# bentotten/radiation_ppo

Hardware: AMD Instinct MI355X
Metric: env steps/sec (whole node) at 4096 envs; PPO iters/sec at 1/2/4/8 GPUs (higher is better)
Workload: dtype f32 policy / f64+int32 env

## Files before the change

### include/radsearch.h

```cpp
#ifndef RADSEARCH_H
#define RADSEARCH_H

#include <stddef.h>
#include <stdint.h>

#ifdef __cplusplus
extern "C" {
#endif

#define RS_ABI_VERSION 4
#define RS_OBS_DIM 11
#define RS_NUM_ACTIONS 9
#define RS_MAX_AGENTS 8
#define RS_MAX_OBS 7

typedef void* rs_stream_t;
typedef struct rs_handle rs_handle;

enum {
    RS_OK = 0,
    RS_ERR_INVALID_ARG = 1,
    RS_ERR_HIP = 2,
    RS_ERR_WORKSPACE = 3,
    RS_ERR_UNSUPPORTED = 4
// ... 22 lines not shown
    int32_t debug_spawn;
} rs_config;

typedef struct rs_info {
    uint8_t* out_of_bounds;
    int32_t* out_of_bounds_count;
    uint8_t* blocked;
    uint8_t* collision;
} rs_info;

const char* rs_strerror(int code);
int rs_abi_version(void);

size_t rs_state_bytes(const rs_config* cfg);

int rs_create(const rs_config* cfg, void* workspace, size_t workspace_bytes, rs_stream_t stream, rs_handle** out);
void rs_destroy(rs_handle* h);

int rs_state_field(rs_handle* h, const char* name, void** dev_ptr, int32_t* elem_bytes, int32_t* rows, int32_t* cols);

int rs_set_epoch_end(rs_handle* h, rs_stream_t stream);

int rs_reset(rs_handle* h, const uint8_t* mask, float* obs, float* reward, float* team, uint8_t* done,
             const rs_info* info, rs_stream_t stream);

int rs_refresh(rs_handle* h, const uint8_t* mask, const int32_t* src_xy, const int32_t* det_xy, const int32_t* intensity,
               const int32_t* bkg, const int32_t* num_obs, const int32_t* rects, float* obs, float* reward, float* team,
               uint8_t* done, const rs_info* info, rs_stream_t stream);

int rs_step(rs_handle* h, const int8_t* actions, float* obs, float* reward, float* team, uint8_t* done,
            const rs_info* info, rs_stream_t stream);

int rs_action_uniforms(rs_handle* h, float* u, rs_stream_t stream);

int rs_error_flags(rs_handle* h, rs_stream_t stream, uint32_t* flags_out);

int rs_gae(const float* rew, const float* val, const uint8_t* cut, const float* last_val, float* adv, float* ret,
           int32_t T, int32_t M, double gamma, double lam, rs_stream_t stream);

size_t rs_ppo_prepare_workspace_bytes(int32_t N);
int rs_ppo_prepare(const uint8_t* cut, const float* adv, float* w, float* adv_n, float* mean_std, void* workspace, int32_t T, int32_t N,
                   int32_t n_total, rs_stream_t stream);

typedef struct rs_mlp_params {
    const float *w1, *b1, *w2, *b2, *w3, *b3;
} rs_mlp_params;

int rs_policy_forward(const rs_mlp_params* actor, const rs_mlp_params* critic, const float* x, int32_t M,
                      float* logits, float* value, rs_stream_t stream);

int rs_ff_team_step(const rs_mlp_params* actors, const rs_mlp_params* critics, int32_t num_agents, const float* x, const float* u,
                    int64_t* act, float* logp_val_boot, int8_t* act8, const uint8_t* mask, int32_t num_envs, rs_stream_t stream);

typedef struct rs_rollout_args {
    int32_t steps_per_epoch;
    int32_t steps_per_episode;
    float* obs;
    int64_t* act;
    float* logp;
    float* val;
    float* rew;
    float* last_val;
    uint8_t* cut;
    float* source_tar;
    float* cur_obs;
    double* w_count;
// ... 306 lines not shown
```

### radiation_ppo_amd/_lib.py

```python
import ctypes as C
import os

import torch

_PKG = os.path.dirname(os.path.abspath(__file__))
LIB_PATH = os.environ.get("RS_LIB_PATH") or os.path.join(_PKG, "lib", "librs_hip.so")

RS_OBS_DIM = 11
RS_MAX_AGENTS = 8
RS_MAX_OBS = 7

ENVERR_ZERO_DIST = 1
ENVERR_IDLE_STALL = 2
ENVERR_CORRECT_CAP = 4
ENVERR_BAD_ACTION = 8
ENVERR_NO_PATH = 16

MAPERR_RING_FULL = 1
MAPERR_VISIT_OVERFLOW = 2
MAPERR_OFF_MAP = 4


class RsConfig(C.Structure):
    _fields_ = [
# ... 44 lines not shown
class RsRolloutArgs(C.Structure):
    _fields_ = [("steps_per_epoch", C.c_int32), ("steps_per_episode", C.c_int32)] + [
        (n, C.c_void_p) for n in ("obs", "act", "logp", "val", "rew", "last_val", "cut", "source_tar", "cur_obs", "w_count",
                                  "w_mean", "w_sq", "w_std", "steps_in_ep", "ep_ret", "done_count", "oob_count",
                                  "ep_ret_sum", "ep_len_sum", "ep_count", "ep_ret_sq_sum", "ep_ret_max", "ep_ret_min")]


class RsPpoBatch(C.Structure):
    _fields_ = [("x", C.c_void_p), ("act", C.c_void_p), ("adv", C.c_void_p), ("ret", C.c_void_p), ("logp_old", C.c_void_p),
                ("w", C.c_void_p), ("M", C.c_int32), ("clip_ratio", C.c_float), ("alpha", C.c_float), ("vf_coef", C.c_float)]


class RsInfo(C.Structure):
    _fields_ = [("out_of_bounds", C.c_void_p), ("out_of_bounds_count", C.c_void_p), ("blocked", C.c_void_p),
                ("collision", C.c_void_p)]


SYMBOLS = [
    ("rs_strerror", C.c_char_p, [C.c_int]),
    ("rs_abi_version", C.c_int, []),
    ("rs_state_bytes", C.c_size_t, [C.POINTER(RsConfig)]),
    ("rs_create", C.c_int, [C.POINTER(RsConfig), C.c_void_p, C.c_size_t, C.c_void_p, C.POINTER(C.c_void_p)]),
    ("rs_destroy", None, [C.c_void_p]),
    ("rs_state_field", C.c_int, [C.c_void_p, C.c_char_p, C.POINTER(C.c_void_p), C.POINTER(C.c_int32),
                                 C.POINTER(C.c_int32), C.POINTER(C.c_int32)]),
    ("rs_set_epoch_end", C.c_int, [C.c_void_p, C.c_void_p]),
    ("rs_reset", C.c_int, [C.c_void_p, C.c_void_p, C.c_void_p, C.c_void_p, C.c_void_p, C.c_void_p,
                           C.POINTER(RsInfo), C.c_void_p]),
    ("rs_refresh", C.c_int, [C.c_void_p, C.c_void_p, C.c_void_p, C.c_void_p, C.c_void_p, C.c_void_p, C.c_void_p, C.c_void_p,
                             C.c_void_p, C.c_void_p, C.c_void_p, C.c_void_p, C.POINTER(RsInfo), C.c_void_p]),
    ("rs_step", C.c_int, [C.c_void_p, C.c_void_p, C.c_void_p, C.c_void_p, C.c_void_p, C.c_void_p,
                          C.POINTER(RsInfo), C.c_void_p]),
    ("rs_action_uniforms", C.c_int, [C.c_void_p, C.c_void_p, C.c_void_p]),
    ("rs_error_flags", C.c_int, [C.c_void_p, C.c_void_p, C.POINTER(C.c_uint32)]),
    ("rs_policy_forward", C.c_int, [C.POINTER(RsMlpParams), C.POINTER(RsMlpParams), C.c_void_p, C.c_int32, C.c_void_p,
                                    C.c_void_p, C.c_void_p]),
    ("rs_ff_team_step", C.c_int, [C.POINTER(RsMlpParams), C.POINTER(RsMlpParams), C.c_int32, C.c_void_p, C.c_void_p, C.c_void_p,
                                  C.c_void_p, C.c_void_p, C.c_void_p, C.c_int32, C.c_void_p]),
    ("rs_rollout", C.c_int, [C.c_void_p, C.POINTER(RsMlpParams), C.POINTER(RsMlpParams), C.POINTER(RsRolloutArgs), C.c_void_p]),
    ("rs_ppo_grad_workspace_bytes", C.c_size_t, []),
    ("rs_ppo_grad", C.c_int, [C.POINTER(RsMlpParams), C.POINTER(RsMlpParams), C.POINTER(RsPpoBatch), C.c_void_p, C.c_void_p,
                              C.c_void_p, C.c_void_p, C.c_void_p]),
    ("rs_adam_step", C.c_int, [C.POINTER(RsMlpParams), C.POINTER(RsMlpParams), C.c_void_p, C.c_void_p, C.c_void_p, C.c_void_p,
                               C.c_void_p, C.c_float, C.c_float, C.c_void_p]),
    ("rs_ppo_update_step", C.c_int, [C.POINTER(RsMlpParams), C.POINTER(RsMlpParams), C.POINTER(RsPpoBatch), C.c_void_p, C.c_void_p,
                                     C.c_void_p, C.c_void_p, C.c_void_p, C.c_void_p, C.c_float, C.c_float, C.c_void_p]),
    ("rs_maps_state_bytes", C.c_size_t, [C.c_int32, C.c_int32, C.c_int32, C.c_int32, C.c_int32]),
    ("rs_maps_create", C.c_int, [C.c_int32, C.c_int32, C.c_int32, C.c_int32, C.c_int32, C.c_double, C.c_void_p, C.c_void_p,
                                 C.c_size_t, C.c_void_p, C.POINTER(C.c_void_p)]),
    ("rs_maps_destroy", None, [C.c_void_p]),
    ("rs_maps_reset", C.c_int, [C.c_void_p, C.c_void_p, C.c_void_p]),
    ("rs_maps_update", C.c_int, [C.c_void_p, C.c_void_p, C.c_void_p, C.c_void_p, C.c_void_p, C.c_void_p]),
    ("rs_maps_stack", C.c_int, [C.c_void_p, C.c_void_p, C.c_void_p, C.c_void_p]),
    ("rs_maps_field", C.c_int, [C.c_void_p, C.c_char_p, C.POINTER(C.c_void_p), C.POINTER(C.c_int32), C.POINTER(C.c_int32),
                                C.POINTER(C.c_int32)]),
    ("rs_cnn_trunk_slab_row", C.c_int32, [C.c_int32]),
    ("rs_cnn_trunk_slab_rows", C.c_int32, [C.c_int64, C.c_int32]),
    ("rs_cnn_trunk_scratch_floats", C.c_int32, [C.c_int32]),
    ("rs_cnn_trunk_forward", C.c_int, [C.c_void_p, C.c_void_p, C.c_void_p, C.c_int32, C.c_int32, C.c_int64, C.c_void_p, C.c_void_p,
                                       C.c_void_p, C.c_void_p, C.c_void_p, C.c_void_p, C.c_void_p, C.c_void_p, C.c_void_p, C.c_void_p]),
    ("rs_cnn_trunk_backward", C.c_int, [C.c_void_p, C.c_void_p, C.c_void_p, C.c_int32, C.c_int32, C.c_int64, C.c_void_p, C.c_void_p,
                                        C.c_void_p, C.c_void_p, C.c_void_p, C.c_void_p, C.c_void_p, C.c_void_p]),
    ("rs_gae", C.c_int, [C.c_void_p, C.c_void_p, C.c_void_p, C.c_void_p, C.c_void_p, C.c_void_p, C.c_int32,
                         C.c_int32, C.c_double, C.c_double, C.c_void_p]),
    ("rs_ppo_prepare_workspace_bytes", C.c_size_t, [C.c_int32]),
    ("rs_ppo_prepare", C.c_int, [C.c_void_p] * 6 + [C.c_int32, C.c_int32, C.c_int32, C.c_void_p]),
# ... 119 lines not shown
```

### radiation_ppo_amd/csrc/rs_device.hpp

```cpp
#pragma once
#include <hip/hip_runtime.h>
#include <stdint.h>

#include "rs_tables.hpp"

#define RS_WAVE 64
#define RS_OBS_DIM 11
#define RS_MAX_AGENTS 8
#define RS_MAX_OBS 7
#define RS_MAX_VERT (4 * RS_MAX_OBS)
#define RS_IDLE 8
#define RS_ACT_NONE 9
#define RS_CORRECT_CAP 4096

#define RS_ENVERR_ZERO_DIST 1u
#define RS_ENVERR_IDLE_STALL 2u
#define RS_ENVERR_CORRECT_CAP 4u
#define RS_ENVERR_BAD_ACTION 8u
#define RS_ENVERR_NO_PATH 16u

#define RS_AF_BLOCKED 1
#define RS_AF_INTERSECT 2
#define RS_AF_OOB 4
#define RS_AF_COLLISION 8
// ... 83 lines not shown
    const double lhs = log(v * invalpha / (a / (us * us) + b));
    const double x = k + 1.0;
    double rhs;
    if (x >= 10.0) {
        const double xi = 1.0 / x, xi2 = xi * xi;
        const double ser = xi * (0.083333333333333333 - xi2 * (0.0027777777777777778 - xi2 * (0.00079365079365079365 - xi2 * 0.00059523809523809524)));
        rhs = k * log(lam / x) - 0.5 * log(x) - lam + x - 0.91893853320467274 - ser;
    } else {
        rhs = -lam + k * log(lam) - lgamma(x);
    }
    return lhs <= rhs;
}

__device__ __forceinline__ int64_t rs_poisson(double lam, uint32_t t, uint32_t episode, uint32_t stream, uint32_t k0, uint32_t k1) {
    if (lam == 0.0) return 0;
    if (lam < 10.0) return rs_poisson_small(lam, t, episode, stream, k0, k1);
    double slam = sqrt(lam);
    double b = 0.931 + 2.53 * slam;
    double a = -0.059 + 0.02483 * b;
    double vr = 0.9277 - 3.6224 / (b - 2.0);
    for (uint32_t i = 0;; ++i) {
        u32x4 o = philox4x32_10(i, t, episode, stream, k0, k1);
        double u = u53(o.x, o.y) - 0.5;
        double v = u53(o.z, o.w);
        double us = 0.5 - fabs(u);
        if (!(us > 0.0)) continue;
        double k = floor((2.0 * a / us + b) * u + lam + 0.43);
        if (us >= 0.07 && v <= vr) return (int64_t)k;
        if (k < 0.0 || (us < 0.013 && v > us)) continue;
        if (rs_ptrs_slow_accept(v, us, k, lam, a, b)) return (int64_t)k;
    }
}

__device__ __forceinline__ double rs_round2(double x) {
    uint64_t bits = (uint64_t)__double_as_longlong(x);
    int ex = (int)((bits >> 52) & 0x7ff);
    if (ex == 0x7ff) return x;
    double sgn = (bits >> 63) ? -1.0 : 1.0;
    if (ex == 0) return sgn * 0.0;
    uint64_t m = (bits & 0xFFFFFFFFFFFFFull) | (1ull << 52);
    int s = 1075 - ex;
    if (s <= 0) return x;
    if (m >= (1ull << 57)) return x;
    uint64_t P = m * 100ull;
    if (s >= 61) return sgn * 0.0;
    uint64_t q = P >> s;
    uint64_t rem = P & ((1ull << s) - 1ull);
    uint64_t half = 1ull << (s - 1);
    if (rem > half || (rem == half && (q & 1ull))) q += 1;
    if (q < 256ull) return sgn * RS_CENT_TAB[q];
    return sgn * ((double)q / 100.0);
}

__device__ __forceinline__ bool rs_isclose_abs(double a, double b, double abs_tol) {
    if (a == b) return true;
    if (isinf(a) || isinf(b)) return false;
    double diff = fabs(b - a);
    return (diff <= fabs(1e-9 * b)) || (diff <= fabs(1e-9 * a)) || (diff <= abs_tol);
}

__device__ __forceinline__ double rs_dist_i(int ax, int ay, int bx, int by) {
    double dx = (double)(ax - bx), dy = (double)(ay - by);
    return sqrt(dx * dx + dy * dy);
}

__device__ __forceinline__ void rs_action_step(int a, int& dx, int& dy) {
// ... 323 lines not shown
__device__ __forceinline__ unsigned long long rs_es_now() {
    unsigned long long t;
    asm volatile("s_memtime %0\n\ts_waitcnt lgkmcnt(0)" : "=s"(t) :: "memory");
    return t;
}
#define RS_ESTAMP_DECL unsigned long long es_last = rs_es_now();
#define RS_ESTAMP(i) do { const unsigned long long t_ = rs_es_now(); \
                          if (__builtin_amdgcn_mbcnt_hi(~0u, __builtin_amdgcn_mbcnt_lo(~0u, 0u)) == 0) atomicAdd(&rs_step_stamp_table[i], t_ - es_last); \
                          es_last = rs_es_now(); } while (0)
#else
#define RS_ESTAMP_DECL
#define RS_ESTAMP(i) do {} while (0)
#endif

struct RsEnvRegs {
    int sx, sy, intensity, bkg, iter_count;
    uint32_t episode, tstep, err;
    bool done;
    __device__ __forceinline__ void load(const RsParams& P, int n) {
        sx = P.src_x[n]; sy = P.src_y[n];
        intensity = P.intensity[n]; bkg = P.bkg[n];
        iter_count = P.iter_count[n];
        episode = P.episode[n] - 1u; tstep = P.tstep[n];
        err = 0;
        done = P.done[n] != 0;
    }
    __device__ __forceinline__ void store(const RsParams& P, int n) {
        P.done[n] = done ? 1 : 0;
        P.iter_count[n] = iter_count;
        P.tstep[n] = tstep;
        if (err) P.err[n] |= err;
        err = 0;
    }
};
struct RsAgentRegs {
    int x, y, oobc;
    double sp, prev;
    uint8_t fl;
    __device__ __forceinline__ void load(const RsParams& P, size_t ia) {
        x = P.ax[ia]; y = P.ay[ia]; sp = P.sp[ia]; prev = P.prev[ia]; oobc = P.oobc[ia]; fl = P.aflags[ia];
    }
    __device__ __forceinline__ void store(const RsParams& P, size_t ia) const {
        P.ax[ia] = x; P.ay[ia] = y; P.sp[ia] = sp; P.prev[ia] = prev; P.oobc[ia] = oobc; P.aflags[ia] = fl;
    }
};

#ifdef RS_STEP_STAMPS
#define RS_ESTAMP_PARAM , unsigned long long& es_last
#define RS_ESTAMP_ARG , es_last
#else
#define RS_ESTAMP_PARAM
#define RS_ESTAMP_ARG
#endif

template <bool HAS_OBS, int CN = 1>
__device__ __forceinline__ void rs_agent_step_core(const RsParams& P, const RsGeo& g, int n, int a, int act, bool collided, RsEnvRegs& E,
                                                   RsAgentRegs& S, const RsOut& O, double& max_reward, bool& have_max, int cj RS_ESTAMP_PARAM) {
    const int N = P.N, A = P.A;
    const int sx = E.sx, sy = E.sy, intensity = E.intensity, bkg = E.bkg;
    const uint32_t episode = E.episode, t = E.tstep;
    const uint32_t k0 = P.seed, k1 = P.env_id_base + (uint32_t)n;
    uint32_t err = 0;
    bool done = E.done;
    if (act < 0) act = RS_IDLE;
    if (act > RS_ACT_NONE) { err |= RS_ENVERR_BAD_ACTION; act = RS_IDLE; }
    int x = S.x, y = S.y;
    double sp = S.sp, prev = S.prev;
    int oobc = S.oobc;
    uint8_t fl = S.fl & (RS_AF_BLOCKED | RS_AF_INTERSECT);
    bool moved = false;
    int px = x, py = y;
    if (act != RS_ACT_NONE) {
        if (collided) {
            fl |= RS_AF_COLLISION;
        } else {
            int dx, dy; rs_action_step(act, dx, dy);
            int tx = x + dx, ty = y + dy;
            bool roll_back = false;
            if (P.enforce) {
                if ((tx < P.bx0 || ty < P.by0) || (P.bx1 <= tx || P.by1 <= ty)) { fl |= RS_AF_OOB; oobc += 1; roll_back = true; }
            } else {
                bool lower_b = x < P.sa_x0 || y < P.sa_y0, upper_b = P.sa_x1 < x || P.sa_y1 < y;
                if (lower_b || upper_b) { fl |= RS_AF_OOB; oobc += 1; }
            }
            if (HAS_OBS && g.n > 0 && rs_in_obstruction(g, tx, ty)) { roll_back = true; fl |= RS_AF_BLOCKED; }
            if (!roll_back) { x = tx; y = ty; px = tx; py = ty; moved = true; }
        }
    }
    RS_ESTAMP(1);
    double euc = rs_dist_i(x, y, sx, sy);
    double reward;
#if defined(RS_ABL) && RS_ABL == 3
    if (moved) sp = euc;
#else
    if (moved) sp = (HAS_OBS && g.n > 0) ? rs_shortest_path<CN>(g, P.dsrc, N, n, sx, sy, x, y, cj) : euc;
#endif
    if (HAS_OBS && !(sp < INFINITY)) err |= RS_ENVERR_NO_PATH;
    RS_ESTAMP(2);
#if defined(RS_ABL) && RS_ABL == 2
    bool inter = false;
#else
    bool inter = (HAS_OBS && g.n > 0) ? rs_is_intersect<CN>(g, px, py, sx, sy, euc, sp, cj) : false;
#endif
    fl = (uint8_t)((fl & ~RS_AF_INTERSECT) | (inter ? RS_AF_INTERSECT : 0));
    RS_ESTAMP(3);
    double lam;
    if (inter) lam = (double)bkg;
    else {
        double r = euc;
        if (r == 0.0) { err |= RS_ENVERR_ZERO_DIST; r = 1.0; }
        lam = (P.falloff ? ((double)intensity / (r * r)) : ((double)intensity / r)) + (double)bkg;
    }
    int64_t meas = rs_poisson(lam, t, episode, RS_STREAM_STEP + (uint32_t)a, k0, k1);
    RS_ESTAMP(4);
    if (moved) {
        if (sp < 110.0) { reward = 0.1; done = true; }
        else if (sp < prev) { reward = 0.1; prev = sp; }
        else reward = ((act == RS_IDLE) ? -1.0 : -0.5) * sp / P.max_dist;
    } else {
        if (act == RS_IDLE && !(fl & RS_AF_COLLISION)) err |= RS_ENVERR_IDLE_STALL;
        reward = -0.5 * sp / P.max_dist;
    }
    reward = rs_round2(reward);
    float* row = O.obs_row + a * RS_OBS_DIM;
    row[0] = (float)(double)meas;
    double nx = 0.0, ny = 0.0;
    if (P.coord_noise) { const RsNoise2 nz = rs_coord_noise(t, episode, (uint32_t)a, k0, k1); nx = nz.x; ny = nz.y; }
    row[1] = (float)(((double)x + nx) * P.scale);
    row[2] = (float)(((double)y + ny) * P.scale);
    RS_ESTAMP(5);
    if ((HAS_OBS && g.n > 0) || P.enforce) rs_sensors<HAS_OBS, CN>(P, g, px, py, row + 3, err, cj);
    else {
#pragma unroll
        for (int i = 0; i < 8; ++i) row[3 + i] = 0.0f;
    }
    RS_ESTAMP(6);
    if (!have_max || max_reward == 0.0) { max_reward = reward; have_max = true; }
    else if (max_reward < reward) max_reward = reward;
    S.x = x; S.y = y; S.sp = sp; S.prev = prev; S.oobc = oobc; S.fl = fl;
    E.done = done; E.err |= err;
    const size_t oa = (size_t)n * A + a;
    if (O.reward) O.reward[oa] = (float)reward;
    if (O.done) O.done[oa] = done ? 1 : 0;
    if (O.oob) O.oob[oa] = (fl & RS_AF_OOB) ? 1 : 0;
    if (O.oobc) O.oobc[oa] = oobc;
    if (O.blocked) O.blocked[oa] = (fl & RS_AF_BLOCKED) ? 1 : 0;
// ... 304 lines not shown
```

### radiation_ppo_amd/csrc/rs_env.hip

```cpp
#include <hip/hip_runtime.h>
#include <stdint.h>
#include <stdlib.h>
#include <string.h>
#include <new>

#include "../../include/radsearch.h"
#include "rs_device.hpp"
#include "rs_handle.hpp"

template <bool HAS_OBS>
__global__ void __launch_bounds__(64, (HAS_OBS ? 4 : 1)) rs_step_kernel(RsParams P, const int8_t* __restrict__ actions, float* obs, RsOut O) {
    extern __shared__ __align__(16) unsigned char smem[];
    int* lds_geo = reinterpret_cast<int*>(smem);
    float* tile = reinterpret_cast<float*>(smem + (HAS_OBS ? RS_MAX_VERT * RS_WAVE * 4 : 0));
    int* flags = reinterpret_cast<int*>(tile + RS_WAVE * rs_tile_stride(P.A));
    const int lane = threadIdx.x & 63;
    const int n = blockIdx.x * blockDim.x + threadIdx.x;
    const bool active = n < P.N;
    RsGeo g{lds_geo, 0, 0, 0};
    if (HAS_OBS) rs_load_geo(P, n, active, lds_geo, g);
    flags[lane] = active ? 1 : 0;
    __syncthreads();
    if (active) {
        RsOut o = O;
// ... 131 lines not shown
            if (flags[l]) dst[i] = tile[l * S + k];
        }
    }
}

template <bool HAS_OBS>
__global__ void __launch_bounds__(64) rs_refresh_kernel(RsParams P, const uint8_t* __restrict__ mask, RsRefresh R, float* obs, RsOut O) {
    extern __shared__ __align__(16) unsigned char smem[];
    constexpr bool has_obs = HAS_OBS;
    int* lds_geo = reinterpret_cast<int*>(smem);
    uint32_t* lds_adj = reinterpret_cast<uint32_t*>(smem + RS_MAX_VERT * RS_WAVE * 4);
    double* lds_d = reinterpret_cast<double*>(smem + 2 * RS_MAX_VERT * RS_WAVE * 4);
    float* tile = reinterpret_cast<float*>(smem + (has_obs ? (2 * RS_MAX_VERT * RS_WAVE * 4 + RS_MAX_VERT * RS_WAVE * 8) : 0));
    int* flags = reinterpret_cast<int*>(tile + RS_WAVE * rs_tile_stride(P.A));
    const int lane = threadIdx.x & 63;
    const int n = blockIdx.x * blockDim.x + threadIdx.x;
    const bool active = n < P.N && (mask == nullptr || mask[n] != 0);
    RsGeo g{lds_geo, 0, 0, 0};
    flags[lane] = active ? 1 : 0;
    __syncthreads();
    if (active) rs_env_refresh_lane<HAS_OBS>(P, g, n, R, lds_geo, lds_adj, lds_d, tile + lane * rs_tile_stride(P.A), O);
    __syncthreads();
    rs_copy_out(P, obs, tile, flags, blockIdx.x * blockDim.x);
}

__global__ void __launch_bounds__(64) rs_action_uniform_kernel(RsParams P, float* __restrict__ u) {
    const int n = blockIdx.x * blockDim.x + threadIdx.x;
    if (n >= P.N) return;
    const uint32_t episode = P.episode[n] - 1u, t = P.tstep[n];
    for (int a = 0; a < P.A; ++a) {
        u32x4 o = philox4x32_10(0u, t, episode, RS_STREAM_ACT + (uint32_t)a, P.seed, P.env_id_base + (uint32_t)n);
        u[(size_t)n * P.A + a] = (float)(o.x >> 8) * (1.0f / 16777216.0f);
    }
}

#define RS_GAE_U 8
__global__ void __launch_bounds__(64) rs_gae_kernel(const float* __restrict__ rew, const float* __restrict__ val,
                                                    const uint8_t* __restrict__ cut, const float* __restrict__ last_val,
                                                    float* __restrict__ adv, float* __restrict__ ret, int T, int M,
                                                    double gamma, double gl, int chunk) {
    const int m = blockIdx.x * blockDim.x + threadIdx.x;
    if (m >= M) return;
    const int t_lo = blockIdx.y * chunk;
    const int t_hi = min(T, t_lo + chunk) - 1;
    if (t_lo >= T) return;
    int t_start = t_hi;
    for (;;) {
        uint8_t cc[16];
#pragma unroll
        for (int u = 0; u < 16; ++u) cc[u] = cut[(size_t)min(t_start + u, T - 1) * M + m];
        int found = -1;
#pragma unroll
        for (int u = 15; u >= 0; --u)
            if (cc[u] != 0 || t_start + u >= T - 1) found = u;
        if (found >= 0) { t_start = min(t_start + found, T - 1); break; }
        t_start += 16;
    }
    double a_acc = 0.0, r_acc = 0.0, v_next = 0.0;
    float r8[RS_GAE_U], v8[RS_GAE_U], l8[RS_GAE_U], rn[RS_GAE_U], vn[RS_GAE_U], ln[RS_GAE_U];
    uint8_t c8[RS_GAE_U], cn[RS_GAE_U];
    auto load_block = [&](int tb, float (&r)[RS_GAE_U], float (&v)[RS_GAE_U], float (&l)[RS_GAE_U], uint8_t (&c)[RS_GAE_U]) {
#pragma unroll
        for (int u = 0; u < RS_GAE_U; ++u) {
            const int t = max(tb - u, t_lo);
            const size_t i = (size_t)t * M + m;
            r[u] = rew[i]; v[u] = val[i]; c[u] = cut[i]; l[u] = last_val[i];
// ... 312 lines not shown
            const rs_info* info, rs_stream_t stream) {
    if (!h || !actions) return RS_ERR_INVALID_ARG;
    hipStream_t s = static_cast<hipStream_t>(stream);
    const RsParams& P = h->P;
    size_t lds = tile_bytes(P.A) + (P.obstruction_count != 0 ? RS_MAX_VERT * RS_WAVE * 4 : 0);
    if (P.obstruction_count != 0) hipLaunchKernelGGL(rs_step4_kernel, dim3((P.N + 15) / 16), dim3(64), lds, s, P, actions, obs, make_out(reward, team, done, info));
    else hipLaunchKernelGGL(rs_step_kernel<false>, dim3((P.N + 63) / 64), dim3(64), lds, s, P, actions, obs, make_out(reward, team, done, info));
    return hipGetLastError() == hipSuccess ? RS_OK : RS_ERR_HIP;
}

int rs_action_uniforms(rs_handle* h, float* u, rs_stream_t stream) {
    if (!h || !u) return RS_ERR_INVALID_ARG;
    const RsParams& P = h->P;
    hipLaunchKernelGGL(rs_action_uniform_kernel, dim3((P.N + 63) / 64), dim3(64), 0, static_cast<hipStream_t>(stream), P, u);
    return hipGetLastError() == hipSuccess ? RS_OK : RS_ERR_HIP;
}

int rs_error_flags(rs_handle* h, rs_stream_t stream, uint32_t* flags_out) {
    if (!h || !flags_out) return RS_ERR_INVALID_ARG;
    hipStream_t s = static_cast<hipStream_t>(stream);
    const int N = h->P.N;
    uint32_t* host = new (std::nothrow) uint32_t[N];
    if (!host) return RS_ERR_HIP;
    int rc = RS_OK;
    if (hipMemcpyAsync(host, h->P.err, sizeof(uint32_t) * (size_t)N, hipMemcpyDeviceToHost, s) != hipSuccess ||
        hipStreamSynchronize(s) != hipSuccess) rc = RS_ERR_HIP;
    uint32_t acc = 0;
    if (rc == RS_OK) for (int i = 0; i < N; ++i) acc |= host[i];
    delete[] host;
    *flags_out = acc;
    return rc;
}

int rs_gae(const float* rew, const float* val, const uint8_t* cut, const float* last_val, float* adv, float* ret,
           int32_t T, int32_t M, double gamma, double lam, rs_stream_t stream) {
    if (!rew || !val || !cut || !last_val || !adv || !ret || T < 1 || M < 1) return RS_ERR_INVALID_ARG;
    hipStream_t s = static_cast<hipStream_t>(stream);
    const int col_waves = (M + 63) / 64;
    int chunks = (512 + col_waves - 1) / col_waves;
    chunks = chunks < 1 ? 1 : (chunks > 16 ? 16 : chunks);
    int chunk = (T + chunks - 1) / chunks;
    if (chunk < 32) chunk = 32;
    chunks = (T + chunk - 1) / chunk;
    hipLaunchKernelGGL(rs_gae_kernel, dim3(col_waves, chunks), dim3(64), 0, s, rew, val, cut, last_val, adv, ret, T, M,
                       gamma, gamma * lam, chunk);
    return hipGetLastError() == hipSuccess ? RS_OK : RS_ERR_HIP;
}

size_t rs_ppo_prepare_workspace_bytes(int32_t N) {
    if (N < 1) return 0;
    return sizeof(double) * ((size_t)(N + 63) / 64 + RS_PREP_BLOCKS);
}

int rs_ppo_prepare(const uint8_t* cut, const float* adv, float* w, float* adv_n, float* mean_std, void* workspace, int32_t T, int32_t N,
                   int32_t n_total, rs_stream_t stream) {
    if (!cut || !adv || !w || !adv_n || !mean_std || !workspace || T < 1 || N < 1 || n_total < 1) return RS_ERR_INVALID_ARG;
    if (reinterpret_cast<uintptr_t>(workspace) & 7u) return RS_ERR_WORKSPACE;
    hipStream_t s = static_cast<hipStream_t>(stream);
    const int col_groups = (N + 63) / 64;
    double* col_sums = static_cast<double*>(workspace);
    double* sq_sums = col_sums + col_groups;
    const size_t n = (size_t)T * (size_t)N;
    const float inv_n_total = (float)(1.0 / (double)n_total);
    hipLaunchKernelGGL(rs_ppo_prepare_cols_kernel, dim3(col_groups), dim3(64), 0, s, cut, adv, w, col_sums, T, N, inv_n_total);
    hipLaunchKernelGGL(rs_ppo_prepare_sq_kernel, dim3(RS_PREP_BLOCKS), dim3(RS_PREP_THREADS), 0, s, adv, col_sums, col_groups, sq_sums, n);
    hipLaunchKernelGGL(rs_ppo_prepare_norm_kernel, dim3(RS_PREP_BLOCKS), dim3(RS_PREP_THREADS), 0, s, adv, col_sums, col_groups, sq_sums, adv_n,
// ... 18 lines not shown
```

### radiation_ppo_amd/csrc/rs_rollout16.hpp

```cpp
#pragma once
#include "rs_mlp.hpp"

__host__ __device__ constexpr int rs_mlp16_lds_floats(int nout) { return 4 * 3 * 64 + 4 * 16 * 64 + 64 + 4 * nout * 16 + nout; }

template <int NOUT>
struct RsMlp16 {
    float* w1f;
    float* w2f;
    float* b2;
    float* w3g;
    float* b3;
    __device__ __forceinline__ void carve(float* base) {
        w1f = base; w2f = w1f + 4 * 3 * 64; b2 = w2f + 4 * 16 * 64; w3g = b2 + 64; b3 = w3g + 4 * NOUT * 16;
    }
    __device__ __forceinline__ void fill(const RsMlpParams& p) {
        const int tid = threadIdx.x, nt = blockDim.x;
        for (int i = tid; i < 4 * 3 * 64; i += nt) {
            const int l = i & 63, s = (i >> 6) % 3, it = i / (3 * 64);
            const int row = 16 * it + (l & 15), k = 4 * s + (l >> 4);
            w1f[i] = RS_TANH_PRESCALE * ((k < RS_IN) ? p.w1[row * RS_IN + k] : p.b1[row]);
        }
        for (int i = tid; i < 4 * 16 * 64; i += nt) {
            const int l = i & 63, ks = (i >> 6) & 15, it = i >> 10;
            const int unit = 16 * (ks >> 2) + 4 * (l >> 4) + (ks & 3);
// ... 97 lines not shown
        for (int i = 0; i < 4; ++i) { pacc[0][i] = 0.0f; pacc[1][i] = 0.0f; }
#pragma unroll
        for (int ut = 0; ut < 4; ++ut)
#pragma unroll
            for (int q = 0; q < 4; ++q) {
                pacc[0] = __builtin_amdgcn_mfma_f32_4x4x1f32(w3[0][4 * ut + q], H2[ut][q], pacc[0], 0, 0, 0);
                pacc[1] = __builtin_amdgcn_mfma_f32_4x4x1f32(w3[1][4 * ut + q], H2[ut][q], pacc[1], 0, 0, 0);
            }
#pragma unroll
        for (int o = 0; o < NOUT; ++o) out[o] = combine(pacc[o >> 2][o & 3], o);
    }
    __device__ __forceinline__ void forward(const float (&xs)[RS_IN_PAD], float (&out)[NOUT]) const {
        f32x4 H2[4];
        Regs none;
        hidden<false>(xs, H2, none);
        output(H2, out);
    }
};

__device__ __forceinline__ void rs_bcast_x16(const float (&xo)[RS_IN_PAD], float (&xs)[RS_IN_PAD]) {
    const int src = threadIdx.x & 15;
#pragma unroll
    for (int k = 0; k < RS_IN_PAD; ++k) xs[k] = __shfl(xo[k], src);
}

constexpr int RS_MB_PRE = 0, RS_MB_POST = 16 * RS_IN_PAD, RS_MB_FLAGS = 2 * 16 * RS_IN_PAD, RS_MB_SLOT = 2 * 16 * RS_IN_PAD + 16;
__host__ __device__ constexpr int rs_rollout16_mailbox_bytes() { return 2 * RS_MB_SLOT * 4; }

#ifdef RS_K6_PARENT_CHAIN
constexpr bool RS_K6_SHORT = false;
#else
constexpr bool RS_K6_SHORT = true;
#endif
template <bool HAS_OBS> struct RsK6Cfg {
    static constexpr bool reg_weights = RS_K6_SHORT && !HAS_OBS;
    static constexpr bool mfma_out = RS_K6_SHORT;
    static constexpr bool reg_state = RS_K6_SHORT;
};

#ifdef RS_K6_STAMPS
#define RS_K6_NPH 16
__device__ unsigned long long rs_k6_stamp_table[2][RS_K6_NPH];
__device__ __forceinline__ unsigned long long rs_k6_now() {
    unsigned long long t;
    asm volatile("s_memtime %0\n\ts_waitcnt lgkmcnt(0)" : "=s"(t) :: "memory");
    return t;
}
#define RS_K6STAMP_DECL unsigned long long k6_acc[RS_K6_NPH] = {0}; const unsigned long long k6_rt0 = __builtin_amdgcn_s_memrealtime(); \
                        unsigned long long k6_last = rs_k6_now();
#define RS_K6STAMP(i) do { __builtin_amdgcn_sched_barrier(0); const unsigned long long t_ = rs_k6_now(); k6_acc[i] += t_ - k6_last; k6_last = t_; \
                           __builtin_amdgcn_sched_barrier(0); } while (0)
#define RS_K6STAMP_EXIT(tmpl, steps) do { if ((threadIdx.x & 63) == 0) { k6_acc[14] = __builtin_amdgcn_s_memrealtime() - k6_rt0; k6_acc[15] = (steps); \
                           for (int q = 0; q < RS_K6_NPH; ++q) atomicAdd(&rs_k6_stamp_table[tmpl][q], k6_acc[q]); } } while (0)
#else
#define RS_K6STAMP_DECL
#define RS_K6STAMP(i) do {} while (0)
#define RS_K6STAMP_EXIT(tmpl, steps) do {} while (0)
#endif

template <bool HAS_OBS>
__global__ void __launch_bounds__(128) rs_rollout16_kernel(RsParams P, RsMlpParams pa, RsMlpParams pc, rs_rollout_args R) {
    extern __shared__ __align__(16) unsigned char smem[];
    float* wts = reinterpret_cast<float*>(smem);
    unsigned char* p = smem + sizeof(float) * (size_t)(rs_mlp16_lds_floats(8) + rs_mlp16_lds_floats(1));
    p = reinterpret_cast<unsigned char*>((reinterpret_cast<uintptr_t>(p) + 15) & ~uintptr_t(15));
    int* lds_geo = reinterpret_cast<int*>(p);
    uint32_t* lds_adj = reinterpret_cast<uint32_t*>(p + RS_MAX_VERT * RS_WAVE * 4);
    double* lds_d = reinterpret_cast<double*>(p + 2 * RS_MAX_VERT * RS_WAVE * 4);
    float* tile = reinterpret_cast<float*>(p + (HAS_OBS ? (2 * RS_MAX_VERT * RS_WAVE * 4 + RS_MAX_VERT * RS_WAVE * 8) : 0));
    float* lds_rew = tile + RS_WAVE * RS_OBS_DIM;
    uint8_t* lds_done = reinterpret_cast<uint8_t*>(lds_rew + RS_WAVE);
    uint8_t* lds_oob = lds_done + RS_WAVE;
    float* mbox = reinterpret_cast<float*>(lds_oob + RS_WAVE);

    RsMlp16<8> ACT; RsMlp16<1> CRT;
    ACT.carve(wts);
    CRT.carve(wts + rs_mlp16_lds_floats(8));
    ACT.fill(pa); CRT.fill(pc);

    const int wave = __builtin_amdgcn_readfirstlane((int)(threadIdx.x >> 6));
    const int lane = threadIdx.x & 63, j = lane & 15;
    const bool own = lane < 16;
    const int n = blockIdx.x * 16 + j;
    const int N = P.N, T = R.steps_per_epoch, L = R.steps_per_episode;
    const int cj = lane >> 4;
    RsGeo g{lds_geo, 0, 0, 0};
    if (HAS_OBS && wave == 0) {
        rs_load_geo(P, n, own, lds_geo, g);
        g.off = __shfl(g.off, j); g.stride = __shfl(g.stride, j); g.n = __shfl(g.n, j);
    }
    __syncthreads();

    if (wave == 1) {
        for (int t = -1; t < T; ++t) {
            __syncthreads();
            const float* M = mbox + (t & 1) * RS_MB_SLOT;
            float xs[RS_IN_PAD];
#pragma unroll
            for (int k = 0; k < RS_IN_PAD; ++k) xs[k] = M[RS_MB_PRE + j * RS_IN_PAD + k];
            float vb;
            { float vv[1]; CRT.forward(xs, vv); vb = vv[0]; }
            const int fl = reinterpret_cast<const int*>(M + RS_MB_FLAGS)[j];
            const bool cut = (fl & 1) != 0, boot = (fl & 2) != 0;
            float v = vb;
            if (__ballot(cut) != 0ull) {
#pragma unroll
                for (int k = 0; k < RS_IN_PAD; ++k) xs[k] = M[RS_MB_POST + j * RS_IN_PAD + k];
                float vv[1];
                CRT.forward(xs, vv);
                v = cut ? vv[0] : vb;
            }
            if (own) {
                if (t >= 0) R.last_val[(size_t)t * N + n] = (cut && boot) ? vb : 0.0f;
                if (t + 1 < T) R.val[(size_t)(t + 1) * N + n] = v;
            }
        }
        return;
    }

    float oraw[RS_OBS_DIM];
#pragma unroll
    for (int k = 0; k < RS_OBS_DIM; ++k) oraw[k] = R.cur_obs[(size_t)n * RS_OBS_DIM + k];
    RsWelford W{R.w_count[n], R.w_mean[n], R.w_sq[n], R.w_std[n]};
    int steps = R.steps_in_ep[n];
    float ep_ret = R.ep_ret[n];
    int done_count = 0, oob_count = 0, ep_count = 0;
    double ep_ret_sum = 0.0, ep_len_sum = 0.0, ep_ret_sq = 0.0;
    float ep_ret_max = -INFINITY, ep_ret_min = INFINITY;
    const uint32_t k0 = P.seed, k1 = P.env_id_base + (uint32_t)n;
// ... 4 lines not shown
    S.load(P, (size_t)n);
    RsMlp16<8>::Regs AR;
    if constexpr (Cfg::reg_weights) ACT.load(AR);

    float xo[RS_IN_PAD], xs[RS_IN_PAD];
#pragma unroll
    for (int k = 0; k < RS_OBS_DIM; ++k) xo[k] = oraw[k];
    xo[0] = W.standardize(oraw[0]);
    xo[11] = 1.0f;
    rs_bcast_x16(xo, xs);
    {
        float* M = mbox + RS_MB_SLOT;
        if (own) {
#pragma unroll
            for (int k = 0; k < RS_IN_PAD; ++k) M[RS_MB_PRE + j * RS_IN_PAD + k] = xo[k];
            reinterpret_cast<int*>(M + RS_MB_FLAGS)[j] = 0;
        }
    }
    __syncthreads();

    RsOut O;
    O.obs_row = tile + j * RS_OBS_DIM;
    O.reward = lds_rew + j - (size_t)n;
    O.team = nullptr;
    O.done = lds_done + j - (size_t)n;
    O.oob = lds_oob + j - (size_t)n;
    O.oobc = nullptr; O.blocked = nullptr; O.collision = nullptr;

    RS_K6STAMP_DECL
    for (int t = 0; t < T; ++t) {
        const size_t row = (size_t)t * N + n;
        float* M = mbox + (t & 1) * RS_MB_SLOT;
        float lg[8];
        {
            f32x4 H2[4];
            ACT.template hidden<Cfg::reg_weights>(xs, H2, AR);
            RS_K6STAMP(0);
            if constexpr (!Cfg::mfma_out) ACT.output(H2, lg);
            else if constexpr (Cfg::reg_weights) ACT.output_mfma(H2, lg, AR.w3);
            else { float w3[2][16]; ACT.load_w3(w3); ACT.output_mfma(H2, lg, w3); }
            RS_K6STAMP(1);
        }
        int a = 0;
        float logp = 0.0f;
        if (own) {
            float mx = lg[0];
#pragma unroll
            for (int q = 1; q < 8; ++q) mx = fmaxf(mx, lg[q]);
            float se = 0.0f;
#pragma unroll
            for (int q = 0; q < 8; ++q) se += __expf(lg[q] - mx);
            const float lse = __logf(se);
            const uint32_t episode = E.episode, tenv = E.tstep;
            u32x4 ph = philox4x32_10(0u, tenv, episode, RS_STREAM_ACT, k0, k1);
            const float u = (float)(ph.x >> 8) * (1.0f / 16777216.0f);
            float cdf = 0.0f;
#pragma unroll
            for (int q = 0; q < 8; ++q) {
                const float lpq = (lg[q] - mx) - lse;
                cdf += __expf(lpq);
                if (q < 7) a += (cdf <= u) ? 1 : 0;
            }
#pragma unroll
            for (int q = 0; q < 8; ++q) logp = (a == q) ? ((lg[q] - mx) - lse) : logp;
#pragma unroll
            for (int k = 0; k < RS_OBS_DIM; ++k) tile[lane * RS_OBS_DIM + k] = xo[k];
        }
        __builtin_amdgcn_wave_barrier();
        RS_K6STAMP(2);
        {
            float* dst = R.obs + ((size_t)t * N + (size_t)blockIdx.x * 16) * RS_OBS_DIM;
            for (int i = lane; i < 16 * RS_OBS_DIM; i += RS_WAVE) dst[i] = tile[i];
        }
        __builtin_amdgcn_wave_barrier();
        bool cut = false;
        bool over = false, boot = false, ended = t == T - 1;
        if (own) {
            R.act[row] = (int64_t)a;
            R.logp[row] = logp;
            R.source_tar[row * 2 + 0] = (float)E.sx;
            R.source_tar[row * 2 + 1] = (float)E.sy;
        }
        RS_K6STAMP(3);
        if (HAS_OBS || own) {
            const int a_env = HAS_OBS ? __shfl(a, j) : a;
            if constexpr (Cfg::reg_state) {
                double max_reward = 0.0;
                bool have_max = false;
#ifdef RS_STEP_STAMPS
                RS_ESTAMP_DECL
#endif
                rs_agent_step_core<HAS_OBS, HAS_OBS ? 4 : 1>(P, g, n, 0, a_env, false, E, S, O, max_reward, have_max, cj RS_ESTAMP_ARG);
            } else {
                rs_env_step_lane<HAS_OBS, HAS_OBS ? 4 : 1>(P, g, n, [&](int) -> int { return a_env; }, O, false, cj);
            }
            E.iter_count += 1;
            E.tstep += 1;
        }
        RS_K6STAMP(4);
        if (own) {
            const float r = lds_rew[lane];
            const bool terminal = lds_done[lane] != 0;
            oob_count += lds_oob[lane];
            R.rew[row] = r;
            ep_ret += r;
            steps += 1;
            done_count += terminal ? 1 : 0;
            const bool timeout = steps == L;
            over = terminal || timeout;
            cut = over || ended;
            boot = timeout || ended;
#pragma unroll
            for (int k = 0; k < RS_OBS_DIM; ++k) oraw[k] = tile[lane * RS_OBS_DIM + k];
            W.update((double)oraw[0]);
#pragma unroll
            for (int k = 1; k < RS_OBS_DIM; ++k) xo[k] = oraw[k];
            xo[0] = W.standardize(oraw[0]);
#pragma unroll
            for (int k = 0; k < RS_IN_PAD; ++k) M[RS_MB_PRE + j * RS_IN_PAD + k] = xo[k];
            reinterpret_cast<int*>(M + RS_MB_FLAGS)[j] = (cut ? 1 : 0) | (boot ? 2 : 0);
            R.cut[row] = cut ? 1 : 0;
            if (over) {
                ep_ret_sum += (double)ep_ret; ep_len_sum += (double)steps; ep_count += 1;
                ep_ret_sq += (double)ep_ret * (double)ep_ret;
                ep_ret_max = fmaxf(ep_ret_max, ep_ret); ep_ret_min = fminf(ep_ret_min, ep_ret);
            }
        }
        RS_K6STAMP(5);
        if (HAS_OBS ? (__shfl((int)cut, j) != 0) : cut) {
            if (ended) P.epoch_end[n] = 1;
            if constexpr (Cfg::reg_state) { S.store(P, (size_t)n); E.store(P, n); }
            if constexpr (HAS_OBS) rs_env_reset_lane<true, 4>(P, g, n, lds_geo, lds_adj, lds_d, tile + j * RS_OBS_DIM, O, j, cj);
            else rs_env_reset_lane<false>(P, g, n, lds_geo, lds_adj, lds_d, tile + lane * RS_OBS_DIM, O);
            E.load(P, n);
            if constexpr (Cfg::reg_state) S.load(P, (size_t)n);
        }
        if (own) {
            if (cut) {
                W.reset();
#pragma unroll
                for (int k = 0; k < RS_OBS_DIM; ++k) oraw[k] = tile[lane * RS_OBS_DIM + k];
                W.update((double)oraw[0]);
#pragma unroll
                for (int k = 1; k < RS_OBS_DIM; ++k) xo[k] = oraw[k];
                xo[0] = W.standardize(oraw[0]);
                steps = 0;
                ep_ret = 0.0f;
#pragma unroll
                for (int k = 0; k < RS_IN_PAD; ++k) M[RS_MB_POST + j * RS_IN_PAD + k] = xo[k];
            }
        }
        RS_K6STAMP(6);
        rs_bcast_x16(xo, xs);
        __syncthreads();
        RS_K6STAMP(7);
    }
    RS_K6STAMP_EXIT(HAS_OBS ? 1 : 0, (unsigned long long)T);
    if constexpr (Cfg::reg_state) {
        if (HAS_OBS || own) { S.store(P, (size_t)n); E.store(P, n); }
    }
    if (own) {
#pragma unroll
        for (int k = 0; k < RS_OBS_DIM; ++k) R.cur_obs[(size_t)n * RS_OBS_DIM + k] = oraw[k];
        R.w_count[n] = W.count; R.w_mean[n] = W.mean; R.w_sq[n] = W.sq; R.w_std[n] = W.std;
        R.steps_in_ep[n] = steps;
        R.ep_ret[n] = ep_ret;
        R.done_count[n] = done_count; R.oob_count[n] = oob_count; R.ep_count[n] = ep_count;
        R.ep_ret_sum[n] = ep_ret_sum; R.ep_len_sum[n] = ep_len_sum;
        R.ep_ret_sq_sum[n] = ep_ret_sq; R.ep_ret_max[n] = ep_ret_max; R.ep_ret_min[n] = ep_ret_min;
// ... 3 lines not shown
```

Measured before the change: 43.63 million.

## Spread Poisson rejection-sampling candidates across wave lane groups and move obs store

The PTRS Poisson draw used in the env step is now evaluated in parallel. The four 16-lane groups of the wave each generate one Philox candidate, the first accepted one is selected by ballot and shuffle, and the code only falls back to a serial loop if none is accepted. The act-stream Philox draw is folded into the same per-group call. Env state is now stepped redundantly on all lanes, and after resets it is broadcast back with shuffles. Observation writes to the rollout buffer move to the top of the next step, read from the mailbox, which removes the tile staging. It also adds a probe kernel and timing stamps to check that grouped and serial draws match, at the cost of extra redundant work on every lane.

```diff
diff --git a/include/radsearch.h b/include/radsearch.h
--- a/include/radsearch.h
+++ b/include/radsearch.h
@@ -78,6 +78,9 @@
             const rs_info* info, rs_stream_t stream);
 
 int rs_action_uniforms(rs_handle* h, float* u, rs_stream_t stream);
+
+int rs_poisson_probe(const double* lam, const uint32_t* t, const uint32_t* episode, const uint32_t* env_id, int64_t count, uint32_t seed,
+                     int64_t* serial, int64_t* group3, int64_t* group4, int32_t* candidates, rs_stream_t stream);
 
 int rs_error_flags(rs_handle* h, rs_stream_t stream, uint32_t* flags_out);
 
diff --git a/radiation_ppo_amd/_lib.py b/radiation_ppo_amd/_lib.py
--- a/radiation_ppo_amd/_lib.py
+++ b/radiation_ppo_amd/_lib.py
@@ -100,6 +100,8 @@
     ("rs_step", C.c_int, [C.c_void_p, C.c_void_p, C.c_void_p, C.c_void_p, C.c_void_p, C.c_void_p,
                           C.POINTER(RsInfo), C.c_void_p]),
     ("rs_action_uniforms", C.c_int, [C.c_void_p, C.c_void_p, C.c_void_p]),
+    ("rs_poisson_probe", C.c_int, [C.c_void_p, C.c_void_p, C.c_void_p, C.c_void_p, C.c_int64, C.c_uint32, C.c_void_p, C.c_void_p,
+                                   C.c_void_p, C.c_void_p, C.c_void_p]),
     ("rs_error_flags", C.c_int, [C.c_void_p, C.c_void_p, C.POINTER(C.c_uint32)]),
     ("rs_policy_forward", C.c_int, [C.POINTER(RsMlpParams), C.POINTER(RsMlpParams), C.c_void_p, C.c_int32, C.c_void_p,
                                     C.c_void_p, C.c_void_p]),
diff --git a/radiation_ppo_amd/csrc/rs_device.hpp b/radiation_ppo_amd/csrc/rs_device.hpp
--- a/radiation_ppo_amd/csrc/rs_device.hpp
+++ b/radiation_ppo_amd/csrc/rs_device.hpp
@@ -139,6 +139,55 @@
     }
 }
 
+struct RsPtrs { double a, b, vr; };
+__device__ __forceinline__ RsPtrs rs_ptrs_setup(double lam) {
+    double slam = sqrt(lam);
+    double b = 0.931 + 2.53 * slam;
+    double a = -0.059 + 0.02483 * b;
+    double vr = 0.9277 - 3.6224 / (b - 2.0);
+    return RsPtrs{a, b, vr};
+}
+__device__ __forceinline__ bool rs_ptrs_try(const u32x4& o, double lam, const RsPtrs& c, double& k) {
+    double u = u53(o.x, o.y) - 0.5;
+    double v = u53(o.z, o.w);
+    double us = 0.5 - fabs(u);
+    if (!(us > 0.0)) return false;
+    k = floor((2.0 * c.a / us + c.b) * u + lam + 0.43);
+    if (us >= 0.07 && v <= c.vr) return true;
+    if (k < 0.0 || (us < 0.013 && v > us)) return false;
+    return rs_ptrs_slow_accept(v, us, k, lam, c.a, c.b);
+}
+template <int FIRST>
+__device__ __forceinline__ int64_t rs_poisson_group(double lam, const u32x4& o, uint32_t t, uint32_t episode, uint32_t stream, uint32_t k0, uint32_t k1) {
+    static_assert(FIRST >= 0 && FIRST < 4, "candidates sit in the lanes g = FIRST..3");
+    const int lane = threadIdx.x & 63, j = lane & 15, g = lane >> 4;
+    const bool ptrs = !(lam == 0.0) && !(lam < 10.0);
+    const RsPtrs c = rs_ptrs_setup(lam);
+    double k = 0.0;
+    const bool acc = ptrs && g >= FIRST && rs_ptrs_try(o, lam, c, k);
+    const unsigned long long won = __ballot(acc) >> j;
+    int src = -1;
+#pragma unroll
+    for (int q = 3; q >= FIRST; --q) src = ((won >> (16 * q)) & 1ull) ? q : src;
+    const int64_t first = __shfl((long long)k, j + 16 * (src < 0 ? 0 : src));
+    if (lam == 0.0) return 0;
+    if (lam < 10.0) return rs_poisson_small(lam, t, episode, stream, k0, k1);
+    if (src >= 0) return first;
+    for (uint32_t i = 4 - FIRST;; ++i) {
+        u32x4 oi = philox4x32_10(i, t, episode, stream, k0, k1);
+        if (rs_ptrs_try(oi, lam, c, k)) return (int64_t)k;
+    }
+}
+__device__ __forceinline__ int rs_poisson_count(double lam, uint32_t t, uint32_t episode, uint32_t stream, uint32_t k0, uint32_t k1) {
+    if (lam == 0.0 || lam < 10.0) return 0;
+    const RsPtrs c = rs_ptrs_setup(lam);
+    double k;
+    for (uint32_t i = 0;; ++i) {
+        u32x4 oi = philox4x32_10(i, t, episode, stream, k0, k1);
+        if (rs_ptrs_try(oi, lam, c, k)) return (int)(i + 1);
+    }
+}
+
 __device__ __forceinline__ double rs_round2(double x) {
     uint64_t bits = (uint64_t)__double_as_longlong(x);
     int ex = (int)((bits >> 52) & 0x7ff);
@@ -528,6 +577,11 @@
         if (err) P.err[n] |= err;
         err = 0;
     }
+    __device__ __forceinline__ void from_lane(int src) {
+        sx = __shfl(sx, src); sy = __shfl(sy, src); intensity = __shfl(intensity, src); bkg = __shfl(bkg, src);
+        iter_count = __shfl(iter_count, src); episode = __shfl(episode, src); tstep = __shfl(tstep, src); err = __shfl(err, src);
+        done = __shfl((int)done, src) != 0;
+    }
 };
 struct RsAgentRegs {
     int x, y, oobc;
@@ -539,11 +593,32 @@
     __device__ __forceinline__ void store(const RsParams& P, size_t ia) const {
         P.ax[ia] = x; P.ay[ia] = y; P.sp[ia] = sp; P.prev[ia] = prev; P.oobc[ia] = oobc; P.aflags[ia] = fl;
     }
+    __device__ __forceinline__ void from_lane(int src) {
+        x = __shfl(x, src); y = __shfl(y, src); oobc = __shfl(oobc, src); sp = __shfl(sp, src); prev = __shfl(prev, src);
+        fl = (uint8_t)__shfl((int)fl, src);
+    }
 };
 
 #ifdef RS_STEP_STAMPS
 #define RS_ESTAMP_PARAM , unsigned long long& es_last
 #define RS_ESTAMP_ARG , es_last
+#elif defined(RS_K6_STAMPS)
+#undef RS_ESTAMP_DECL
+#define RS_ESTAMP_DECL unsigned long long k6p[3] = {0, 0, 0};
+#define RS_ESTAMP_PARAM , unsigned long long (&k6p)[3]
+#define RS_ESTAMP_ARG , k6p
+__device__ __forceinline__ unsigned long long rs_k6p_now() {
+    unsigned long long t;
+    __builtin_amdgcn_sched_barrier(0);
+    asm volatile("s_memtime %0\n\ts_waitcnt lgkmcnt(0)" : "=s"(t) :: "memory");
+    __builtin_amdgcn_sched_barrier(0);
+    return t;
+}
+__device__ __forceinline__ int rs_k6p_wave_max(int v) {
+#pragma unroll
+    for (int off = 32; off > 0; off >>= 1) v = max(v, __shfl_xor(v, off));
+    return v;
+}
 #else
 #define RS_ESTAMP_PARAM
 #define RS_ESTAMP_ARG
@@ -551,7 +626,8 @@
 
 template <bool HAS_OBS, int CN = 1>
 __device__ __forceinline__ void rs_agent_step_core(const RsParams& P, const RsGeo& g, int n, int a, int act, bool collided, RsEnvRegs& E,
-                                                   RsAgentRegs& S, const RsOut& O, double& max_reward, bool& have_max, int cj RS_ESTAMP_PARAM) {
+                                                   RsAgentRegs& S, const RsOut& O, double& max_reward, bool& have_max, int cj RS_ESTAMP_PARAM,
+                                                   const u32x4* cand = nullptr) {
     const int N = P.N, A = P.A;
     const int sx = E.sx, sy = E.sy, intensity = E.intensity, bkg = E.bkg;
     const uint32_t episode = E.episode, t = E.tstep;
@@ -607,7 +683,19 @@
         if (r == 0.0) { err |= RS_ENVERR_ZERO_DIST; r = 1.0; }
         lam = (P.falloff ? ((double)intensity / (r * r)) : ((double)intensity / r)) + (double)bkg;
     }
-    int64_t meas = rs_poisson(lam, t, episode, RS_STREAM_STEP + (uint32_t)a, k0, k1);
+#if defined(RS_K6_STAMPS) && !defined(RS_STEP_STAMPS)
+    const unsigned long long k6p_t0 = rs_k6p_now();
+#endif
+    int64_t meas = cand ? rs_poisson_group<1>(lam, *cand, t, episode, RS_STREAM_STEP + (uint32_t)a, k0, k1)
+                        : rs_poisson(lam, t, episode, RS_STREAM_STEP + (uint32_t)a, k0, k1);
+#if defined(RS_K6_STAMPS) && !defined(RS_STEP_STAMPS)
+    {
+        const unsigned long long t1 = rs_k6p_now();
+        k6p[0] += t1 - k6p_t0;
+        k6p[1] = (unsigned long long)rs_poisson_count(lam, t, episode, RS_STREAM_STEP + (uint32_t)a, k0, k1);
+        k6p[2] += rs_k6p_now() - t1;
+    }
+#endif
     RS_ESTAMP(4);
     if (moved) {
         if (sp < 110.0) { reward = 0.1; done = true; }
diff --git a/radiation_ppo_amd/csrc/rs_env.hip b/radiation_ppo_amd/csrc/rs_env.hip
--- a/radiation_ppo_amd/csrc/rs_env.hip
+++ b/radiation_ppo_amd/csrc/rs_env.hip
@@ -187,6 +187,24 @@
         u32x4 o = philox4x32_10(0u, t, episode, RS_STREAM_ACT + (uint32_t)a, P.seed, P.env_id_base + (uint32_t)n);
         u[(size_t)n * P.A + a] = (float)(o.x >> 8) * (1.0f / 16777216.0f);
     }
+}
+
+__global__ void __launch_bounds__(64) rs_poisson_probe_kernel(const double* __restrict__ lam_in, const uint32_t* __restrict__ t_in,
+                                                              const uint32_t* __restrict__ ep_in, const uint32_t* __restrict__ id_in,
+                                                              long long count, uint32_t seed, int64_t* __restrict__ serial,
+                                                              int64_t* __restrict__ group3, int64_t* __restrict__ group4,
+                                                              int32_t* __restrict__ candidates) {
+    const int lane = threadIdx.x & 63, g = lane >> 4;
+    const long long d = (long long)blockIdx.x * 16 + (lane & 15);
+    const bool live = d < count;
+    double lam = live ? lam_in[d] : 0.0;
+    if (!(lam >= 0.0 && lam <= 1e12)) lam = 0.0;
+    const uint32_t t = live ? t_in[d] : 0u, ep = live ? ep_in[d] : 0u, k1 = live ? id_in[d] : 0u;
+    const int64_t s = rs_poisson(lam, t, ep, RS_STREAM_STEP, seed, k1);
+    const int c = rs_poisson_count(lam, t, ep, RS_STREAM_STEP, seed, k1);
+    const int64_t g3 = rs_poisson_group<1>(lam, philox4x32_10(g ? (uint32_t)(g - 1) : 0u, t, ep, RS_STREAM_STEP, seed, k1), t, ep, RS_STREAM_STEP, seed, k1);
+    const int64_t g4 = rs_poisson_group<0>(lam, philox4x32_10((uint32_t)g, t, ep, RS_STREAM_STEP, seed, k1), t, ep, RS_STREAM_STEP, seed, k1);
+    if (live && g == 0) { serial[d] = s; group3[d] = g3; group4[d] = g4; candidates[d] = c; }
 }
 
 #define RS_GAE_U 8
@@ -565,6 +583,15 @@
     return rc;
 }
 
+int rs_poisson_probe(const double* lam, const uint32_t* t, const uint32_t* episode, const uint32_t* env_id, int64_t count, uint32_t seed,
+                     int64_t* serial, int64_t* group3, int64_t* group4, int32_t* candidates, rs_stream_t stream) {
+    if (!lam || !t || !episode || !env_id || !serial || !group3 || !group4 || !candidates || count < 1 || count > (int64_t)1 << 34)
+        return RS_ERR_INVALID_ARG;
+    hipLaunchKernelGGL(rs_poisson_probe_kernel, dim3((unsigned)((count + 15) / 16)), dim3(64), 0, static_cast<hipStream_t>(stream), lam, t,
+                       episode, env_id, (long long)count, seed, serial, group3, group4, candidates);
+    return hipGetLastError() == hipSuccess ? RS_OK : RS_ERR_HIP;
+}
+
 int rs_gae(const float* rew, const float* val, const uint8_t* cut, const float* last_val, float* adv, float* ret,
            int32_t T, int32_t M, double gamma, double lam, rs_stream_t stream) {
     if (!rew || !val || !cut || !last_val || !adv || !ret || T < 1 || M < 1) return RS_ERR_INVALID_ARG;
diff --git a/radiation_ppo_amd/csrc/rs_rollout16.hpp b/radiation_ppo_amd/csrc/rs_rollout16.hpp
--- a/radiation_ppo_amd/csrc/rs_rollout16.hpp
+++ b/radiation_ppo_amd/csrc/rs_rollout16.hpp
@@ -153,10 +153,20 @@
 #else
 constexpr bool RS_K6_SHORT = true;
 #endif
+#ifdef RS_K6_SERIAL_DRAW
+constexpr bool RS_K6_GROUP = false;
+#else
+constexpr bool RS_K6_GROUP = true;
+#endif
+#ifndef RS_K6_OBS_BY_WAVE1
+#define RS_K6_OBS_BY_WAVE1 true
+#endif
 template <bool HAS_OBS> struct RsK6Cfg {
     static constexpr bool reg_weights = RS_K6_SHORT && !HAS_OBS;
     static constexpr bool mfma_out = RS_K6_SHORT;
     static constexpr bool reg_state = RS_K6_SHORT;
+    static constexpr bool group_draw = RS_K6_GROUP && reg_state;
+    static constexpr bool obs_by_wave1 = RS_K6_SHORT && RS_K6_GROUP && RS_K6_OBS_BY_WAVE1 && !HAS_OBS;
 };
 
 #ifdef RS_K6_STAMPS
@@ -168,14 +178,18 @@
     return t;
 }
 #define RS_K6STAMP_DECL unsigned long long k6_acc[RS_K6_NPH] = {0}; const unsigned long long k6_rt0 = __builtin_amdgcn_s_memrealtime(); \
-                        unsigned long long k6_last = rs_k6_now();
+                        unsigned long long k6_last = rs_k6_now(); unsigned long long k6p[3] = {0, 0, 0};
 #define RS_K6STAMP(i) do { __builtin_amdgcn_sched_barrier(0); const unsigned long long t_ = rs_k6_now(); k6_acc[i] += t_ - k6_last; k6_last = t_; \
                            __builtin_amdgcn_sched_barrier(0); } while (0)
-#define RS_K6STAMP_EXIT(tmpl, steps) do { if ((threadIdx.x & 63) == 0) { k6_acc[14] = __builtin_amdgcn_s_memrealtime() - k6_rt0; k6_acc[15] = (steps); \
+#define RS_K6STAMP_TRIPS(active) do { const int m_ = rs_k6p_wave_max((active) ? (int)k6p[1] : 0); k6_acc[9] += m_; k6_acc[10] += m_ > 3 ? m_ - 3 : 0; } while (0)
+#define RS_K6STAMP_PHILOX(t0) do { k6_acc[12] += rs_k6p_now() - (t0); } while (0)
+#define RS_K6STAMP_EXIT(tmpl, steps) do { if ((threadIdx.x & 63) == 0) { k6_acc[8] = k6p[0]; k6_acc[11] = k6p[2]; k6_acc[14] = __builtin_amdgcn_s_memrealtime() - k6_rt0; k6_acc[15] = (steps); \
                            for (int q = 0; q < RS_K6_NPH; ++q) atomicAdd(&rs_k6_stamp_table[tmpl][q], k6_acc[q]); } } while (0)
 #else
 #define RS_K6STAMP_DECL
 #define RS_K6STAMP(i) do {} while (0)
+#define RS_K6STAMP_TRIPS(active) do {} while (0)
+#define RS_K6STAMP_PHILOX(t0) do {} while (0)
 #define RS_K6STAMP_EXIT(tmpl, steps) do {} while (0)
 #endif
 
@@ -216,6 +230,16 @@
         for (int t = -1; t < T; ++t) {
             __syncthreads();
             const float* M = mbox + (t & 1) * RS_MB_SLOT;
+            if constexpr (RsK6Cfg<HAS_OBS>::obs_by_wave1) {
+                if (t + 1 < T) {
+                    float* dst = R.obs + ((size_t)(t + 1) * N + (size_t)blockIdx.x * 16) * RS_OBS_DIM;
+                    const int* F = reinterpret_cast<const int*>(M + RS_MB_FLAGS);
+                    for (int i = lane; i < 16 * RS_OBS_DIM; i += RS_WAVE) {
+                        const int e = i / RS_OBS_DIM, k = i - e * RS_OBS_DIM;
+                        dst[i] = M[((F[e] & 1) ? RS_MB_POST : RS_MB_PRE) + e * RS_IN_PAD + k];
+                    }
+                }
+            }
             float xs[RS_IN_PAD];
 #pragma unroll
             for (int k = 0; k < RS_IN_PAD; ++k) xs[k] = M[RS_MB_PRE + j * RS_IN_PAD + k];
@@ -286,6 +310,15 @@
         const size_t row = (size_t)t * N + n;
         float* M = mbox + (t & 1) * RS_MB_SLOT;
         float lg[8];
+        u32x4 ph{0u, 0u, 0u, 0u};
+        if constexpr (Cfg::group_draw) {
+#ifdef RS_K6_STAMPS
+            const unsigned long long p0 = rs_k6p_now();
+#endif
+            ph = philox4x32_10(cj ? (uint32_t)(cj - 1) : 0u, E.tstep, E.episode, cj ? RS_STREAM_STEP : RS_STREAM_ACT, k0, k1);
+            RS_K6STAMP_PHILOX(p0);
+            RS_K6STAMP(13);
+        }
         {
             f32x4 H2[4];
             ACT.template hidden<Cfg::reg_weights>(xs, H2, AR);
@@ -305,8 +338,13 @@
 #pragma unroll
             for (int q = 0; q < 8; ++q) se += __expf(lg[q] - mx);
             const float lse = __logf(se);
-            const uint32_t episode = E.episode, tenv = E.tstep;
-            u32x4 ph = philox4x32_10(0u, tenv, episode, RS_STREAM_ACT, k0, k1);
+            if constexpr (!Cfg::group_draw) {
+#ifdef RS_K6_STAMPS
+                const unsigned long long p0 = rs_k6p_now();
+#endif
+                ph = philox4x32_10(0u, E.tstep, E.episode, RS_STREAM_ACT, k0, k1);
+                RS_K6STAMP_PHILOX(p0);
+            }
             const float u = (float)(ph.x >> 8) * (1.0f / 16777216.0f);
             float cdf = 0.0f;
 #pragma unroll
@@ -317,12 +355,14 @@
             }
 #pragma unroll
             for (int q = 0; q < 8; ++q) logp = (a == q) ? ((lg[q] - mx) - lse) : logp;
-#pragma unroll
-            for (int k = 0; k < RS_OBS_DIM; ++k) tile[lane * RS_OBS_DIM + k] = xo[k];
+            if constexpr (!Cfg::obs_by_wave1) {
+#pragma unroll
+                for (int k = 0; k < RS_OBS_DIM; ++k) tile[lane * RS_OBS_DIM + k] = xo[k];
+            }
         }
         __builtin_amdgcn_wave_barrier();
         RS_K6STAMP(2);
-        {
+        if constexpr (!Cfg::obs_by_wave1) {
             float* dst = R.obs + ((size_t)t * N + (size_t)blockIdx.x * 16) * RS_OBS_DIM;
             for (int i = lane; i < 16 * RS_OBS_DIM; i += RS_WAVE) dst[i] = tile[i];
         }
@@ -336,21 +376,24 @@
             R.source_tar[row * 2 + 1] = (float)E.sy;
         }
         RS_K6STAMP(3);
-        if (HAS_OBS || own) {
-            const int a_env = HAS_OBS ? __shfl(a, j) : a;
+        constexpr bool STEP_ALL = HAS_OBS || Cfg::group_draw;
+        if (STEP_ALL || own) {
+            const int a_env = STEP_ALL ? __shfl(a, j) : a;
             if constexpr (Cfg::reg_state) {
                 double max_reward = 0.0;
                 bool have_max = false;
 #ifdef RS_STEP_STAMPS
                 RS_ESTAMP_DECL
 #endif
-                rs_agent_step_core<HAS_OBS, HAS_OBS ? 4 : 1>(P, g, n, 0, a_env, false, E, S, O, max_reward, have_max, cj RS_ESTAMP_ARG);
+                rs_agent_step_core<HAS_OBS, HAS_OBS ? 4 : 1>(P, g, n, 0, a_env, false, E, S, O, max_reward, have_max, cj RS_ESTAMP_ARG,
+                                                             Cfg::group_draw ? &ph : nullptr);
             } else {
                 rs_env_step_lane<HAS_OBS, HAS_OBS ? 4 : 1>(P, g, n, [&](int) -> int { return a_env; }, O, false, cj);
             }
             E.iter_count += 1;
             E.tstep += 1;
         }
+        RS_K6STAMP_TRIPS(STEP_ALL || own);
         RS_K6STAMP(4);
         if (own) {
             const float r = lds_rew[lane];
@@ -389,6 +432,9 @@
             E.load(P, n);
             if constexpr (Cfg::reg_state) S.load(P, (size_t)n);
         }
+        if constexpr (Cfg::group_draw && !HAS_OBS) {
+            if (__ballot(cut) != 0ull) { E.from_lane(j); S.from_lane(j); }
+        }
         if (own) {
             if (cut) {
                 W.reset();
```

Result: faster. 44.24 million, median of 6 (+1.4%).
